# NTT123/vietTTS

Hardware: AMD Instinct MI355X
Metric: audio samples/sec whole-node, HiFi-GAN V1 mel2wave (higher is better)
Workload: dtype bf16; 1 GPU; HiFi-GAN V1 generator, 64 utterances x 1024 mel frames per GPU per step (BASELINE configs[2] shape), bf16; batch_per_gpu=64, frames=1024, parallelism=dp1 utterance-sharded, weights broadcast once, no data-path collective, microbatch=0, streams=0, schedule=engine default: micro-batches of <= 32768 frames on two HIP streams

## Files before the change

viettts_amd/csrc/engine.hip:

```cpp
#include "../../include/vtts_hifigan.h"

#include <hip/hip_runtime.h>

#include <cmath>
#include <cstdarg>
#include <cstdio>
#include <cstring>
#include <string>
#include <vector>

#include "vtts_internal.h"

using namespace vtts;

namespace {

thread_local std::string g_last_error;

}

int vtts::failf(int code, const char* fmt, ...) {
    char buf[512];
    va_list ap;
    va_start(ap, fmt);
    vsnprintf(buf, sizeof(buf), fmt, ap);
    va_end(ap);
    g_last_error = buf;
    return code;
}

namespace {

enum Kind { KIND_CONV = 0, KIND_CONVT = 1 };

struct Layer {
    std::string key;
    int kind = KIND_CONV;
    int cin = 0, cout = 0, k = 0, dil = 1, stride = 1;
    int pad = 0;
    int pad_a = 0;
    std::vector<float> w, b;
    bool have_w = false, have_b = false;
    size_t off_w = 0, off_b = 0, off_wp = 0;
    bool has_wp = false;
    size_t wp_floats = 0;
    int bcls = BCLS_NONE;
    size_t off_wb = 0, wb_bytes = 0;
    int coutp = 0;
    bool has_pair = false;
    size_t off_pw = 0, pw_bytes = 0, off_pb = 0;
    bool has_rb = false;
    size_t off_rw = 0, rw_bytes = 0, off_rb = 0;
    bool has_ug = false;
    size_t off_ug = 0, ug_bytes = 0;
    bool has_x3 = false;
    size_t off_x3 = 0;
};

}

struct vtts_hifigan {
    vtts_hifigan_cfg cfg;
    int device = 0;
    int dtype = VTTS_F32;
    bool x3 = false;
    int hop = 1;
    std::vector<Layer> layers;
    int idx_pre = -1, idx_post = -1;
    std::vector<int> idx_ups;
    std::vector<int> idx_res;
    size_t blob_bytes = 0;
    char* blob = nullptr;
    int64_t opt_kernels = 0;
    int64_t opt_microbatch = 0;
    int64_t opt_profile = 0;
    int cur_b0 = 0;
    const int* cur_lens = nullptr;
    int cur_T = 0;
    int64_t opt_tiles = 0;
    int64_t opt_fuse = 2;
    int64_t opt_streams = 0;
    int64_t opt_graph = 1;
    struct GraphEntry {
        const void* mel = nullptr;
        void* wav = nullptr;
        void* ws = nullptr;
        int B = 0, T = 0, seen = 0;
        uint64_t epoch = 0, last_use = 0;
        hipGraph_t graph = nullptr;
        hipGraphExec_t exec = nullptr;
    };
    std::vector<GraphEntry> graphs;
    hipStream_t cap_stream = nullptr;
    uint64_t epoch = 0, use_clock = 0;
    int64_t opt_zigzag = 1;
    unsigned zrev_count = 0;
    int64_t opt_tail = 1;
    int64_t opt_chains = 1;
    hipEvent_t ev_chain[3] = {nullptr, nullptr, nullptr};
    hipStream_t side_streams[3] = {nullptr, nullptr, nullptr};
    hipEvent_t ev_fork = nullptr, ev_join[3] = {nullptr, nullptr, nullptr};
    int prof_C = 0, prof_K = 0;
    std::vector<std::pair<hipEvent_t, hipEvent_t>> prof_events;
    size_t prof_used = 0;
    double prof_flops = 0.0;
    std::string prof_name, prof_name_pair;
};

namespace {

int conv_same_pad_a(int k, int s) {
    const int pad_len = k + s - 2;
    return (s > k - 1) ? (k - 1) : (pad_len + 1) / 2;
}

void pick_dominant_class(vtts_hifigan* h, bool mfma_only) {
    double best_flops = -1.0;
    for (const Layer& l : h->layers) {
        if (&l == &h->layers[h->idx_pre] || l.kind != KIND_CONV || l.cin != l.cout || (mfma_only && !l.has_wp)) continue;
        double fl = 0.0;
        long len2 = 1;
        for (auto& m : h->layers) {
            if (m.kind == KIND_CONVT) len2 *= m.stride;
            if (m.kind == KIND_CONV && m.cin == l.cin && m.k == l.k && m.cin == m.cout) fl += 2.0 * len2 * m.cin * m.cout * m.k;
        }
        if (fl > best_flops) {
            best_flops = fl;
            h->prof_C = l.cin;
            h->prof_K = l.k;
        }
    }
}

bool dominant(const vtts_hifigan* h, const Layer& l) {
    return l.kind == KIND_CONV && l.cin == h->prof_C && l.cout == h->prof_C && l.k == h->prof_K;
}

int classify_bf16(const vtts_hifigan* h, const Layer& l, bool is_pre, bool is_post) {
    if (is_post) return (l.cin == 32 && l.cout == 1 && l.k == 7) ? BCLS_NONE - 1 : BCLS_NONE;
    if (is_pre) return (l.cin <= 128 && l.cin % 8 == 0 && l.cout == 512 && l.k == 7) ? BCLS_PRE : BCLS_NONE;
    if (l.kind == KIND_CONVT) {
        if (!convT1d_f32_mfma_supported(l.cin, l.cout, l.k, l.stride, l.pad_a, 4)) return BCLS_NONE;
        if (l.cin == 512) return BCLS_UP0;
        if (l.cin == 256) return BCLS_UP1;
        if (l.cin == 128) return BCLS_UP2;
        return BCLS_UP3;
    }
    if (l.cin != l.cout || !(l.k == 3 || l.k == 7 || l.k == 11) || l.dil > 5) return BCLS_NONE;
    switch (l.cin) {
        case 256: return BCLS_RES256;
        case 128: return BCLS_RES128;
        case 64: return BCLS_RES64;
        case 32: return BCLS_RES32;
    }
    return BCLS_NONE;
}

int build_layers_bf16(vtts_hifigan* h) {
    size_t off = 0;
    for (auto& l : h->layers) {
        const bool is_pre = (&l == &h->layers[h->idx_pre]), is_post = (&l == &h->layers[h->idx_post]);
        l.bcls = classify_bf16(h, l, is_pre, is_post);
        if (l.bcls == BCLS_NONE)
            return failf(VTTS_ERR_INVALID, "dtype bf16: no kernel for module %s (%d->%d, k=%d): the bf16 path covers the HiFi-GAN V1 shapes",
                         l.key.c_str(), l.cin, l.cout, l.k);
        l.coutp = (l.kind == KIND_CONVT) ? l.cout * l.stride : l.cout;
        l.off_b = off;
        off = align_up(off + (size_t)l.coutp * sizeof(float), 256);
        if (is_post) {
            l.off_w = off;
            off = align_up(off + (size_t)l.k * l.cin * l.cout * sizeof(float), 256);
        } else {
            const BPackGeom g = bf16_pack_geom(l.bcls, l.kind == KIND_CONVT ? 3 : l.k);
            l.wb_bytes = bf16_packed_bytes(g);
            l.off_wb = off;
            off = align_up(off + l.wb_bytes, 256);
            if (l.kind == KIND_CONVT || (is_pre && l.bcls == BCLS_PRE && l.cin == 80)) {
                l.has_ug = true;
                l.ug_bytes = bf16_packed_bytes(convt_g_pack_geom(l.bcls));
                l.off_ug = off;
// ... 323 lines not shown
    const ConvArgs a = resblock_args(h, rb[0], x, B, L, y, acc_mode, div);
    const int dils[3] = {rb[0].dil, rb[2].dil, rb[4].dil};
    const void* w[6];
    const float* bias[6];
    for (int q = 0; q < 6; ++q) {
        w[q] = h->blob + rb[q].off_x3;
        bias[q] = reinterpret_cast<const float*>(h->blob + rb[q].off_b);
    }
    return launch_timed(h, rb[0], 6, B, L, s, "split-operand ResBlock launch", [&] { return launch_resblock_x3(a, dils, w, bias, s); });
}

int run_layer_bf16(vtts_hifigan* h, const Layer& l, const void* x, int x_pitch, int cin_real, int B, int L, float slope_in,
                   float slope_out, const void* res, void* y, int acc_add, float div, hipStream_t s) {
    BConvArgs a;
    memset(&a, 0, sizeof(a));
    a.x = x;
    a.wp = h->blob + l.off_wb;
    a.bias = reinterpret_cast<const float*>(h->blob + l.off_b);
    a.res = res;
    a.y = y;
    a.B = B;
    a.L = L;
    set_ragged(h, a, L);
    a.x_pitch = x_pitch;
    a.cin_real = cin_real;
    a.dil = (l.kind == KIND_CONVT) ? 1 : l.dil;
    a.pad = (l.kind == KIND_CONVT) ? 1 : l.pad;
    a.convt_halves = (l.kind == KIND_CONVT) ? 1 : 0;
    a.slope_in = slope_in;
    a.slope_out = slope_out;
    a.acc_add = acc_add;
    a.div = div;
    const int K = (l.kind == KIND_CONVT) ? 3 : l.k;
    const bool ug = (l.kind == KIND_CONVT || l.bcls == BCLS_PRE) && l.has_ug && h->opt_fuse >= 1 && res == nullptr && acc_add == 0 && div == 1.0f;
    if (ug) a.wp = h->blob + l.off_ug;
    if (ug) a.zrev = next_zrev(h);
    return launch_timed(h, l, 1, B, L, s, "bf16 kernel launch",
                        [&] { return ug ? launch_convt_g_bf16(l.bcls, a, s) : launch_conv_bf16(l.bcls, K, a, s); });
}

BConvArgs resblock_args_bf16(vtts_hifigan* h, const Layer& c1, const void* x, int B, int L, float slope_out, void* y, int acc_add, float div) {
    BConvArgs a;
    memset(&a, 0, sizeof(a));
    a.x = x;
    a.y = y;
    a.B = B;
    a.L = L;
    set_ragged(h, a, L);
    a.x_pitch = c1.cin;
    a.cin_real = c1.cin;
    a.slope_in = 0.1f;
    a.slope_out = slope_out;
    a.acc_add = acc_add;
    a.div = div;
    a.zrev = next_zrev(h);
    return a;
}

int run_pair_bf16(vtts_hifigan* h, const Layer& c1, const void* x, int B, int L, float slope_out, void* y, int acc_add, float div,
                  hipStream_t s, float* tail_wav = nullptr) {
    BConvArgs a = resblock_args_bf16(h, c1, x, B, L, slope_out, y, acc_add, div);
    a.wp = h->blob + c1.off_pw;
    a.bias = reinterpret_cast<const float*>(h->blob + c1.off_pb);
    a.dil = c1.dil;
    a.pad = c1.pad;
    a.tile_pref = (int)h->opt_tiles;
    if (tail_wav) {
        const Layer& post = h->layers[h->idx_post];
        a.tail_wav = tail_wav;
        a.tail_wf = reinterpret_cast<const float*>(h->blob + post.off_w);
        a.tail_bias = reinterpret_cast<const float*>(h->blob + post.off_b);
    }
    return launch_timed(h, c1, 2, B, L, s, "fused pair launch", [&] { return launch_pair_g_bf16(c1.cin, c1.k, a, s); });
}

int run_resblock_bf16(vtts_hifigan* h, const Layer* rb, const void* x, int B, int L, float slope_out, void* y, int acc_add, float div,
                      hipStream_t s) {
    BConvArgs a = resblock_args_bf16(h, rb[0], x, B, L, slope_out, y, acc_add, div);
    a.wp = h->blob + rb[0].off_rw;
    a.bias = reinterpret_cast<const float*>(h->blob + rb[0].off_rb);
    a.dils[0] = rb[0].dil;
    a.dils[1] = rb[2].dil;
    a.dils[2] = rb[4].dil;
    return launch_timed(h, rb[0], 0, B, L, s, "fused ResBlock launch", [&] { return launch_resblock_bf16(rb[0].cin, rb[0].k, a, s); });
}

Route route_bf16(const vtts_hifigan* h, const Layer* rb) {
    if (h->opt_fuse >= 2 && rb[0].has_rb && (h->opt_fuse >= 3 || resblock_bf16_preferred(rb[0].cin, rb[0].k))) return ROUTE_RESBLOCK;
    if (h->opt_fuse >= 1 && rb[0].has_pair && rb[2].has_pair && rb[4].has_pair) return ROUTE_PAIRS;
    return ROUTE_CONVS;
}

bool tail_fused_bf16(const vtts_hifigan* h) {
    if (!h->opt_tail || h->cfg.resblock == 2) return false;
    const Layer* rb = &h->layers[h->idx_res.back()];
    const Layer& post = h->layers[h->idx_post];
    return route_bf16(h, rb) == ROUTE_PAIRS && pair_tail_bf16_supported(rb[0].cin, rb[0].k, post.cin, post.cout, post.k);
}

size_t elem_bytes(const vtts_hifigan* h) { return h->dtype == VTTS_BF16 ? 2 : sizeof(float); }

size_t max_act_elems(const vtts_hifigan* h, int T) {
    size_t best = (size_t)h->cfg.upsample_initial_channel * T;
    long L = T;
    for (int i = 0; i < h->cfg.num_upsamples; ++i) {
        L *= h->cfg.upsample_rates[i];
        size_t e = (size_t)(h->cfg.upsample_initial_channel >> (i + 1)) * L;
        if (e > best) best = e;
    }
    return best;
}

int auto_streams(const vtts_hifigan* h) { return h->opt_streams > 0 ? (int)h->opt_streams : 2; }

int pass_frames(const vtts_hifigan* h) { return (h->dtype == VTTS_F32 && auto_streams(h) >= 2) ? 32768 : 65536; }

int microbatch_frames(const vtts_hifigan* h) { return auto_streams(h) >= 2 ? 32768 : 65536; }

int pick_microbatch(const vtts_hifigan* h, int B, int T) {
    if (h->opt_microbatch > 0) return (int)std::min<int64_t>(h->opt_microbatch, B);
    const int frames = microbatch_frames(h);
    int mb = (frames + T - 1) / T;
    if (mb < 1) mb = 1;
    if (mb > B) mb = B;
    int nmb = (B + mb - 1) / mb;
    const int ns = auto_streams(h);
    if (nmb > 1 && ns > 1) nmb = (nmb + ns - 1) / ns * ns;
    if (nmb > B) nmb = B;
    mb = (B + nmb - 1) / nmb;
    return mb;
}

int check_pass_size(const vtts_hifigan* h, int B, int T) {
    const size_t bytes = max_act_elems(h, T) * elem_bytes(h);
    if (bytes >= ((size_t)1 << 31))
        return failf(VTTS_ERR_INVALID, "T=%d frames is too long for one pass (%zu activation bytes per utterance, limit 2^31): synthesize it in chunks",
                     T, bytes);
    if (pick_microbatch(h, B, T) > 65535) return failf(VTTS_ERR_INVALID, "at most 65535 utterances per pass (got %d)", B);
    return VTTS_OK;
}

constexpr int PAR_CHAIN_FRAMES = 2048;

struct PassBufs {
    char *X = nullptr, *S = nullptr;
    char *T[VTTS_MAX_KERNELS] = {}, *C[VTTS_MAX_KERNELS] = {}, *Y[VTTS_MAX_KERNELS] = {};
};

struct PassPlan {
    int mb = 1, nstr = 1, nbuf = 4;
    size_t es = 0, per = 0;
    bool par = false;
    int chain_bufs = 0;

    size_t bytes() const { return (size_t)nstr * nbuf * per; }
    PassBufs buffers(void* ws, int si, int nk) const {
        char* slot = static_cast<char*>(ws) + (size_t)si * nbuf * per;
        auto at = [&](int q) { return slot + (size_t)q * per; };
        PassBufs b;
        b.X = at(0);
        b.S = at(par ? 1 : 3);
        for (int j = 0; j < nk; ++j) {
            b.T[j] = par ? at(2 + chain_bufs * j) : at(1);
            b.C[j] = par ? at(3 + chain_bufs * j) : at(2);
            if (par && chain_bufs == 3) b.Y[j] = at(4 + 3 * j);
        }
        return b;
// ... 649 lines not shown
    }
};

VTTS_API int vtts_hifigan_run_module(vtts_hifigan* h, const char* key, const float* x_dev, int B, int L, float slope_in,
                                     const float* res_dev, float* y_dev, vtts_stream stream) {
    if (!h || !key || !x_dev || !y_dev) return failf(VTTS_ERR_INVALID, "null argument");
    if (!h->blob) return failf(VTTS_ERR_STATE, "run_module() before pack()/bind_packed()");
    if (B <= 0 || L <= 0) return failf(VTTS_ERR_INVALID, "B and L must be positive");
    Layer* l = find_layer(h, key);
    if (!l) return failf(VTTS_ERR_INVALID, "unknown module '%s'", key);
    const bool is_pre = (l == &h->layers[h->idx_pre]);
    const bool is_post = (l == &h->layers[h->idx_post]);
    if (h->dtype == VTTS_BF16) {
        if (!(slope_in > 0.0f && slope_in <= 1.0f)) return failf(VTTS_ERR_INVALID, "run_module(): slope_in must lie in (0, 1] on a bf16 handle (got %g)", slope_in);
        hipStream_t st = static_cast<hipStream_t>(stream);
        const size_t nx = (size_t)B * L * l->cin, ny = (size_t)B * L * (l->kind == KIND_CONVT ? l->stride : 1) * l->cout;
        DevBuf xbuf, rbuf, ybuf;
        void *&xb = xbuf.p, *&rb = rbuf.p, *&yb = ybuf.p;
        int rc = VTTS_OK;
        if (is_post) {
            HIP_TRY(hipMalloc(&xb, nx * 2));
            if (launch_f32_to_bf16(x_dev, xb, nx, st) != hipSuccess) rc = failf(VTTS_ERR_HIP, "conversion launch failed");
            BConvArgs a;
            memset(&a, 0, sizeof(a));
            a.x = xb;
            a.wf = reinterpret_cast<const float*>(h->blob + l->off_w);
            a.bias = reinterpret_cast<const float*>(h->blob + l->off_b);
            a.B = B;
            a.L = L;
            if (!rc && launch_conv_post_bf16(a, y_dev, nullptr, st) != hipSuccess) rc = failf(VTTS_ERR_HIP, "conv_post launch failed");
        } else {
            HIP_TRY(hipMalloc(&yb, ny * 2));
            if (!is_pre) {
                HIP_TRY(hipMalloc(&xb, nx * 2));
                if (launch_f32_to_bf16(x_dev, xb, nx, st) != hipSuccess) rc = failf(VTTS_ERR_HIP, "conversion launch failed");
            }
            if (res_dev) {
                HIP_TRY(hipMalloc(&rb, ny * 2));
                if (launch_f32_to_bf16(res_dev, rb, ny, st) != hipSuccess) rc = failf(VTTS_ERR_HIP, "conversion launch failed");
            }
            if (!rc) rc = run_layer_bf16(h, *l, is_pre ? static_cast<const void*>(x_dev) : xb, l->cin, l->cin, B, L, slope_in, 1.0f, rb, yb, 0, 1.f, st);
            if (!rc && launch_bf16_to_f32(yb, y_dev, ny, st) != hipSuccess) rc = failf(VTTS_ERR_HIP, "conversion launch failed");
        }
        hipError_t e = hipStreamSynchronize(st);
        if (!rc && e != hipSuccess) rc = failf(VTTS_ERR_HIP, "run_module failed: %s", hipGetErrorString(e));
        return rc;
    }
    Act x = is_pre ? Act{x_dev, (long)L * l->cin, 1, l->cin} : Act{x_dev, (long)l->cin * L, L, 1};
    return run_layer(h, *l, x, B, L, slope_in, res_dev, y_dev, ACC_STORE, 1.f, is_post ? 1 : 0, nullptr,
                     static_cast<hipStream_t>(stream));
}

VTTS_API int vtts_hifigan_run_pair(vtts_hifigan* h, const char* key_c1, const float* x_dev, int B, int L, float* y_dev, vtts_stream stream) {
    if (!h || !key_c1 || !x_dev || !y_dev) return failf(VTTS_ERR_INVALID, "null argument");
    if (!h->blob) return failf(VTTS_ERR_STATE, "run_pair() before pack()/bind_packed()");
    if (B <= 0 || L <= 0) return failf(VTTS_ERR_INVALID, "B and L must be positive");
    Layer* l = find_layer(h, key_c1);
    const Layer* c2 = l && l + 1 < h->layers.data() + h->layers.size() ? l + 1 : nullptr;
    if (h->dtype == VTTS_F32) {
        const bool x3 = c2 && pair_x3_wanted(h, *l, *c2, L);
        if (!x3 && (!c2 || !pair_f32_fusable(*l, *c2, L)))
            return failf(VTTS_ERR_INVALID, "'%s' is not the first convolution of a ResBlock pair the fused fp32 kernel covers (C in {32, 64, 128}, L a multiple of 4)", key_c1);
        return run_pair_f32(h, *l, *c2, x3, x_dev, B, L, y_dev, ACC_STORE, 1.f, static_cast<hipStream_t>(stream));
    }
    if (!l || !l->has_pair) return failf(VTTS_ERR_INVALID, "'%s' is not the first convolution of a fused ResBlock pair", key_c1);
    hipStream_t st = static_cast<hipStream_t>(stream);
    const size_t n = (size_t)B * L * l->cin;
    DevBuf xbuf, ybuf;
    void *&xb = xbuf.p, *&yb = ybuf.p;
    HIP_TRY(hipMalloc(&xb, n * 2));
    HIP_TRY(hipMalloc(&yb, n * 2));
    int rc = VTTS_OK;
    if (launch_f32_to_bf16(x_dev, xb, n, st) != hipSuccess) rc = failf(VTTS_ERR_HIP, "conversion launch failed");
    if (!rc) rc = run_pair_bf16(h, *l, xb, B, L, 1.0f, yb, 0, 1.f, st);
    if (!rc && launch_bf16_to_f32(yb, y_dev, n, st) != hipSuccess) rc = failf(VTTS_ERR_HIP, "conversion launch failed");
    hipError_t e = hipStreamSynchronize(st);
    if (!rc && e != hipSuccess) rc = failf(VTTS_ERR_HIP, "run_pair failed: %s", hipGetErrorString(e));
    return rc;
}

VTTS_API int vtts_hifigan_set_option(vtts_hifigan* h, const char* name, int64_t value) {
    if (!h || !name) return failf(VTTS_ERR_INVALID, "null argument");
    {
        static const char* const writable[] = {"kernels", "microbatch", "fuse", "streams", "graph", "zigzag", "chains", "tiles", "tail", "stage"};
        for (const char* w : writable) {
            int64_t cur = 0;
            if (!strcmp(name, w) && vtts_hifigan_get_option(h, name, &cur) == VTTS_OK && cur == value) return VTTS_OK;
        }
    }
    ++h->epoch;
    if (!strcmp(name, "kernels")) {
        if (value != 0 && value != 1) return failf(VTTS_ERR_INVALID, "kernels must be 0 (auto) or 1 (generic)");
        h->opt_kernels = value;
    } else if (!strcmp(name, "microbatch")) {
        if (value < 0) return failf(VTTS_ERR_INVALID, "microbatch must be >= 0");
        h->opt_microbatch = value;
    } else if (!strcmp(name, "fuse")) {
        if (value < 0 || value > 3) return failf(VTTS_ERR_INVALID, "fuse must be 0 (per convolution), 1 (pairs), 2 (bf16: pairs + whole ResBlocks where faster; fp32: pairs at C <= 64) or 3 (... wherever supported)");
        h->opt_fuse = value;
    } else if (!strcmp(name, "streams")) {
        if (value < 0 || value > 4) return failf(VTTS_ERR_INVALID, "streams must be 1..4 (0 = the engine's default)");
        h->opt_streams = value;
    } else if (!strcmp(name, "graph")) {
        if (value != 0 && value != 1) return failf(VTTS_ERR_INVALID, "graph must be 0 (always eager) or 1 (small launches replay a captured hipGraph)");
        h->opt_graph = value;
    } else if (!strcmp(name, "zigzag")) {
        if (value != 0 && value != 1) return failf(VTTS_ERR_INVALID, "zigzag must be 0 or 1");
        h->opt_zigzag = value;
    } else if (!strcmp(name, "chains")) {
        if (value < 0 || value > 2) return failf(VTTS_ERR_INVALID, "chains must be 0 (ResBlocks of a stage one after the other), 1 (side by side on small fp32 launches) or 2 (... on every single-micro-batch launch)");
        h->opt_chains = value;
    } else if (!strcmp(name, "tiles")) {
        if (value < 0 || value > 2) return failf(VTTS_ERR_INVALID, "tiles must be 0 (auto), 1 (wide) or 2 (narrow)");
        h->opt_tiles = value;
    } else if (!strcmp(name, "tail")) {
        if (value != 0 && value != 1) return failf(VTTS_ERR_INVALID, "tail must be 0 or 1");
        h->opt_tail = value;
    } else if (!strcmp(name, "stage")) {
        if (value != 0) return failf(VTTS_ERR_INVALID, "stage must be 0: the whole-stage kernel was removed (it measured slower, profiles/r06_a_stage_kernel_findings.md)");
    } else if (!strcmp(name, "profile")) {
        h->opt_profile = value ? 1 : 0;
    } else if (!strcmp(name, "hop") || !strcmp(name, "pass_frames") || !strcmp(name, "max_frames_per_pass") || !strcmp(name, "graphs_cached") ||
               !strcmp(name, "profile_C") || !strcmp(name, "profile_K")) {
        return failf(VTTS_ERR_INVALID, "option '%s' is read-only", name);
    } else {
        return failf(VTTS_ERR_INVALID, "unknown option '%s'", name);
    }
    return VTTS_OK;
}

VTTS_API int vtts_hifigan_get_option(const vtts_hifigan* h, const char* name, int64_t* value) {
    if (!h || !name || !value) return failf(VTTS_ERR_INVALID, "null argument");
    if (!strcmp(name, "kernels")) *value = h->opt_kernels;
    else if (!strcmp(name, "microbatch")) *value = h->opt_microbatch;
    else if (!strcmp(name, "profile")) *value = h->opt_profile;
    else if (!strcmp(name, "tiles")) *value = h->opt_tiles;
    else if (!strcmp(name, "streams")) *value = h->opt_streams;
    else if (!strcmp(name, "zigzag")) *value = h->opt_zigzag;
    else if (!strcmp(name, "chains")) *value = h->opt_chains;
    else if (!strcmp(name, "graph")) *value = h->opt_graph;
    else if (!strcmp(name, "tail")) *value = h->opt_tail;
    else if (!strcmp(name, "stage")) *value = 0;
    else if (!strcmp(name, "graphs_cached")) {
        *value = 0;
        for (auto& g : h->graphs) *value += g.exec ? 1 : 0;
    }
    else if (!strcmp(name, "fuse")) *value = h->opt_fuse;
    else if (!strcmp(name, "hop")) *value = h->hop;
    else if (!strcmp(name, "max_frames_per_pass")) {
        const size_t per = max_act_elems(h, 1) * elem_bytes(h);
        *value = (int64_t)((((size_t)1 << 31) + per - 1) / per);
    }
    else if (!strcmp(name, "pass_frames")) *value = pass_frames(h);
    else if (!strcmp(name, "profile_C")) *value = h->prof_C;
    else if (!strcmp(name, "profile_K")) *value = h->prof_K;
    else return failf(VTTS_ERR_INVALID, "unknown option '%s'", name);
    return VTTS_OK;
}

VTTS_API int vtts_hifigan_profile_read(vtts_hifigan* h, double* resblock_ms, int64_t* launches, double* resblock_flops,
                                       int reset) {
    if (!h) return failf(VTTS_ERR_INVALID, "null argument");
    double ms = 0.0;
    for (size_t i = 0; i < h->prof_used; ++i) {
        float t = 0.f;
        HIP_TRY(hipEventSynchronize(h->prof_events[i].second));
        HIP_TRY(hipEventElapsedTime(&t, h->prof_events[i].first, h->prof_events[i].second));
        ms += t;
    }
    if (resblock_ms) *resblock_ms = ms;
    if (launches) *launches = (int64_t)h->prof_used;
    if (resblock_flops) *resblock_flops = h->prof_flops;
    if (reset) {
        h->prof_used = 0;
        h->prof_flops = 0.0;
    }
    return VTTS_OK;
}

VTTS_API const char* vtts_hifigan_profile_kernel(const vtts_hifigan* h) {
    if (!h) return "";
    return (h->dtype == VTTS_BF16 && h->opt_fuse) ? h->prof_name_pair.c_str() : h->prof_name.c_str();
}
```

viettts_amd/csrc/kernels_bf16_rbk.hip:

```cpp
#include <string.h>

#include <type_traits>

#include "bf16_common.h"

#ifndef VTTS_WREG_RB_MAX
#define VTTS_WREG_RB_MAX 64
#endif

namespace vtts {

template <int C_, int KS_, int W_, int WM_, int WN_, int PA_, int MINWG_>
struct RBTile {
    static constexpr int C = C_, KS = KS_, W = W_, WM = WM_, WN = WN_, PA = PA_, MINWG = MINWG_;
    static constexpr int THREADS = 64 * WM * WN, MR = C / WM / 32, NR = W / WN / 32;
    static constexpr int H = (KS - 1) / 2;
    static constexpr int MAXDIL = 5;
    static constexpr int GUARD = H * MAXDIL;
    static constexpr int ROWS = W + 2 * GUARD;
    static constexpr int SPR = C / 8, P = C * 2;
    static constexpr int KSTEPS = C / 16;
    static constexpr int NQT = KS * KSTEPS;
    static constexpr int MB = C / 32;
    static constexpr int RA = PA + 1;
    static constexpr int TILE_BYTES = tile_rows16(ROWS) * P;
    static constexpr int BIAS_BYTES = 6 * C * 4;
    static constexpr int LDS_BYTES = 2 * TILE_BYTES + BIAS_BYTES;
    static constexpr size_t CONV_BYTES = (size_t)KS * C * C * 2;
    static constexpr int XPT = (W * SPR + THREADS - 1) / THREADS;
    static_assert(C % (WM * 32) == 0 && W % (WN * 32) == 0 && LDS_BYTES <= 160 * 1024, "window / LDS");
    static_assert(RA == 4 && (NQT % 4 == 0 || NQT % 4 == 2), "ring of 4; a phase starts at slot 0 or 2");
    static constexpr bool WREG = NQT * MR * 4 <= VTTS_WREG_RB_MAX;
};

template <class T>
__global__ __launch_bounds__(T::THREADS, (T::MINWG * T::THREADS + 255) / 256) void resblock_bf16_k(BConvArgs a) {
    constexpr int C = T::C, KS = T::KS, W = T::W, PA = T::PA, RA = T::RA, MR = T::MR, NR = T::NR, H = T::H, GUARD = T::GUARD;
    constexpr int THREADS = T::THREADS, SPR = T::SPR, P = T::P, KSTEPS = T::KSTEPS, NQT = T::NQT, XPT = T::XPT, MB = T::MB;

    extern __shared__ __attribute__((aligned(16))) unsigned char lds[];
    unsigned char* tA = lds;
    unsigned char* tT = lds + T::TILE_BYTES;
    const float* sbias = reinterpret_cast<const float*>(lds + 2 * T::TILE_BYTES);

    const int tid = threadIdx.x;
    const int lane = tid & 63;
    const int wave = tid >> 6;
    const int wm = wave / T::WN, wn = wave % T::WN;
    const int cb0 = wm * (C / T::WM);
    const int l31 = lane & 31;
    const int lh = lane >> 5;
    const int b = a.zrev ? (int)(gridDim.z - 1 - blockIdx.z) : (int)blockIdx.z;
    const int Lp = a.L;
    const int L = a.lens ? min(max(a.lens[b], 0) * a.len_mul, a.L) : a.L;
    const int d0 = a.dils[0], d1 = a.dils[1], d2 = a.dils[2];
    const int M = H * (d0 + d1 + d2) + 3 * H;
    const int NT = W - 2 * M;
    const int ntv = (L + NT - 1) / NT, rx = (int)((blockIdx.x + b) & 7), lox = (rx * ntv) >> 3, hix = ((rx + 1) * ntv) >> 3;
    const bool xmap = (a.L + NT - 1) / NT >= 192;
    const int tile = xmap ? lox + (int)(blockIdx.x >> 3) : (int)blockIdx.x;
    if (xmap && tile >= hix) return;
    const int t0 = tile * NT;
    if (t0 >= L) return;
    const int tw = t0 - M;
    const unsigned short* __restrict__ xg = static_cast<const unsigned short*>(a.x) + (size_t)b * Lp * C;
    unsigned short* __restrict__ yg = static_cast<unsigned short*>(a.y) + (size_t)b * Lp * C;

    auto act2 = [](unsigned u) { return lrelu01_pack(bf16_lo(u), bf16_hi(u)); };

    for (int u = tid; u < 6 * C; u += THREADS) reinterpret_cast<float*>(lds + 2 * T::TILE_BYTES)[u] = a.bias[u];
    for (int u = tid; u < 2 * 2 * GUARD * SPR; u += THREADS) {
        const int tile = u / (2 * GUARD * SPR), v = u % (2 * GUARD * SPR);
        const int gr = v % (2 * GUARD), c = v / (2 * GUARD);
        const int row = gr < GUARD ? gr : W + gr;
        *reinterpret_cast<uint4*>((tile ? tT : tA) + tile_off<SPR>(row, c)) = make_uint4(0u, 0u, 0u, 0u);
    }
    {
        constexpr int RPI = THREADS / SPR;
        static_assert(THREADS % SPR == 0 && RPI % 16 == 0 && (W * SPR) % THREADS == 0, "a thread's units share their column and their swizzle");
        constexpr int RW = 64 / SPR;
        const int r0 = SPR >= 16 ? tid / SPR : wave * RW + lane % RW, c = SPR >= 16 ? tid % SPR : lane / RW;
        unsigned char* const lds0 = tA + tile_off<SPR>(GUARD + r0, c);
        uint4 v[XPT];
        if (tw >= 0 && tw + W <= L) {
            const unsigned short* __restrict__ g0 = xg + (size_t)(tw + r0) * C + c * 8;
#pragma unroll
            for (int i = 0; i < XPT; ++i) v[i] = *reinterpret_cast<const uint4*>(g0 + (size_t)i * RPI * C);
        } else {
#pragma unroll
            for (int i = 0; i < XPT; ++i) {
                const int t = tw + r0 + i * RPI;
                const int tc = t < 0 ? 0 : (t >= L ? L - 1 : t);
                v[i] = *reinterpret_cast<const uint4*>(xg + (size_t)tc * C + c * 8);
                if (t < 0 || t >= L) v[i] = make_uint4(0u, 0u, 0u, 0u);
            }
        }
#pragma unroll
        for (int i = 0; i < XPT; ++i) {
            v[i].x = act2(v[i].x);
            v[i].y = act2(v[i].y);
            v[i].z = act2(v[i].z);
            v[i].w = act2(v[i].w);
        }
#pragma unroll
        for (int i = 0; i < XPT; ++i) *reinterpret_cast<uint4*>(lds0 + i * RPI * P) = v[i];
    }
    const int col0 = wn * (W / T::WN) + l31;
    uint4 xr[MR][NR][2];
#pragma unroll
    for (int mr = 0; mr < MR; ++mr)
#pragma unroll
        for (int nr = 0; nr < NR; ++nr)
#pragma unroll
            for (int p = 0; p < 2; ++p) {
                const int t = tw + col0 + nr * 32;
// ... 61 lines not shown
            }
        };
        constexpr int TAILQ = NQT % 4;
        load_b(0, 0);
        __builtin_amdgcn_sched_group_barrier(0x100, NR, 0);
#pragma nounroll
        for (int q0 = 0; q0 < NQT - 4 - TAILQ; q0 += 4) {
#pragma unroll
            for (int i = 0; i < 4; ++i) step(q0 + i, i, true);
        }
        if constexpr (TAILQ == 0) {
#pragma unroll
            for (int i = 0; i < 4; ++i) step(NQT - 4 + i, i, i < 3);
        } else {
#pragma unroll
            for (int i = 0; i < 4; ++i) step(NQT - 6 + i, i, true);
            step(NQT - 2, 0, true);
            step(NQT - 1, 1, false);
        }
    };
    constexpr int NQW = T::WREG ? NQT : 1;
    bf16x8 aw[NQW][MR];
    auto load_w_all = [&](int conv) {
        if constexpr (T::WREG) {
            if (conv < 6) {
#pragma unroll
                for (int q = 0; q < NQT; ++q)
#pragma unroll
                    for (int mr = 0; mr < MR; ++mr) aw[q][mr] = __builtin_bit_cast(bf16x8, aptr[(size_t)((conv * NQT + q) * MB + mr) * 64]);
            }
        }
    };
    auto conv_phase_wreg = [&](const unsigned char* __restrict__ tile, int dl, int conv) {
        f32x16 bblk[MR];
#pragma unroll
        for (int mr = 0; mr < MR; ++mr)
#pragma unroll
            for (int rq = 0; rq < 4; ++rq) {
                const float4 bv = *reinterpret_cast<const float4*>(sbias + conv * C + cb0 + 32 * mr + 8 * rq + 4 * lh);
                bblk[mr][4 * rq + 0] = bv.x;
                bblk[mr][4 * rq + 1] = bv.y;
                bblk[mr][4 * rq + 2] = bv.z;
                bblk[mr][4 * rq + 3] = bv.w;
            }
        bf16x8 bf[2][NR];
        auto load_b = [&](int q, int par) {
            const int tap = q / KSTEPS, ks = q % KSTEPS;
#pragma unroll
            for (int nr = 0; nr < NR; ++nr) bf[par][nr] = *reinterpret_cast<const bf16x8*>(tile + tile_off<SPR>(GUARD + col0 + nr * 32 + (tap - H) * dl, ks * 2 + lh));
        };
        load_b(0, 0);
        __builtin_amdgcn_sched_group_barrier(0x100, NR, 0);
#pragma unroll
        for (int q = 0; q < NQT; ++q) {
            if (q + 1 < NQT) load_b(q + 1, (q + 1) & 1);
#pragma unroll
            for (int mr = 0; mr < MR; ++mr)
#pragma unroll
                for (int nr = 0; nr < NR; ++nr)
                    acc[mr][nr] = __builtin_amdgcn_mfma_f32_32x32x16_bf16(aw[q < NQW ? q : 0][mr], bf[q & 1][nr], q == 0 ? bblk[mr] : acc[mr][nr], 0, 0, 0);
            for (int i = 0; i < MR * NR; ++i) {
                __builtin_amdgcn_sched_group_barrier(0x008, 1, 0);
                if (q + 1 < NQT && i < NR) __builtin_amdgcn_sched_group_barrier(0x100, 1, 0);
            }
        }
    };
    if constexpr (T::WREG) {
        load_w_all(0);
    } else {
#pragma unroll
        for (int q = 0; q < PA; ++q) load_a(q, q % RA);
    }
    const bool interior = tw >= 0 && tw + W <= L;
    auto write_tile = [&](unsigned char* tile, int mr, int nr, unsigned p0, unsigned p1, unsigned q0, unsigned q1, int p) {
        const int row = GUARD + col0 + nr * 32;
        const int t = tw + col0 + nr * 32;
        if (!interior && (t < 0 || t >= L)) p0 = p1 = q0 = q1 = 0u;
        swap_pair(p0, q0);
        swap_pair(p1, q1);
        const int slot = ((cb0 + 32 * mr) >> 3) + 2 * p + lh;
        *reinterpret_cast<uint4*>(tile + tile_off<SPR>(row, slot)) = make_uint4(p0, p1, q0, q1);
    };

    __syncthreads();
    if constexpr (!T::WREG) init_acc(0);

    constexpr int S2 = NQT % 4;
#pragma nounroll
    for (int pr = 0; pr < 3; ++pr) {
        const int dl = pr == 0 ? d0 : (pr == 1 ? d1 : d2);
        if constexpr (T::WREG) {
            conv_phase_wreg(tA, dl, 2 * pr);
            load_w_all(2 * pr + 1);
        } else {
            conv_phase(2 * pr, std::integral_constant<int, 0>{}, tA, dl);
        }
#pragma unroll
        for (int mr = 0; mr < MR; ++mr)
#pragma unroll
            for (int nr = 0; nr < NR; ++nr)
#pragma unroll
                for (int p = 0; p < 2; ++p) {
                    const int r0 = 8 * p;
                    const f32x16& c = acc[mr][nr];
                    write_tile(tT, mr, nr, lrelu01_pack(c[r0 + 0], c[r0 + 1]), lrelu01_pack(c[r0 + 2], c[r0 + 3]),
                               lrelu01_pack(c[r0 + 4], c[r0 + 5]), lrelu01_pack(c[r0 + 6], c[r0 + 7]), p);
                }
        if constexpr (!T::WREG) init_acc(2 * pr + 1);
        __syncthreads();
        if constexpr (T::WREG) {
            conv_phase_wreg(tT, 1, 2 * pr + 1);
            load_w_all(2 * pr + 2);
        } else {
            conv_phase(2 * pr + 1, std::integral_constant<int, S2>{}, tT, 1);
        }
#pragma unroll
        for (int mr = 0; mr < MR; ++mr)
#pragma unroll
            for (int nr = 0; nr < NR; ++nr)
#pragma unroll
                for (int p = 0; p < 2; ++p) {
                    const int r0 = 8 * p;
                    const uint4 r = xr[mr][nr][p];
                    f32x16& c = acc[mr][nr];
                    c[r0 + 0] = vadd_raw(bf16_lo(r.x), c[r0 + 0]); c[r0 + 1] = vadd_raw(bf16_hi(r.x), c[r0 + 1]);
                    c[r0 + 2] = vadd_raw(bf16_lo(r.y), c[r0 + 2]); c[r0 + 3] = vadd_raw(bf16_hi(r.y), c[r0 + 3]);
                    c[r0 + 4] = vadd_raw(bf16_lo(r.z), c[r0 + 4]); c[r0 + 5] = vadd_raw(bf16_hi(r.z), c[r0 + 5]);
                    c[r0 + 6] = vadd_raw(bf16_lo(r.w), c[r0 + 6]); c[r0 + 7] = vadd_raw(bf16_hi(r.w), c[r0 + 7]);
                }
        if (pr < 2) {
#pragma unroll
            for (int mr = 0; mr < MR; ++mr)
#pragma unroll
                for (int nr = 0; nr < NR; ++nr)
#pragma unroll
                    for (int p = 0; p < 2; ++p) {
                        const int r0 = 8 * p;
                        const f32x16& c = acc[mr][nr];
                        uint4 r;
                        r.x = pack_bf16x2(c[r0 + 0], c[r0 + 1]);
                        r.y = pack_bf16x2(c[r0 + 2], c[r0 + 3]);
                        r.z = pack_bf16x2(c[r0 + 4], c[r0 + 5]);
                        r.w = pack_bf16x2(c[r0 + 6], c[r0 + 7]);
                        xr[mr][nr][p] = r;
                        write_tile(tA, mr, nr, act2(r.x), act2(r.y), act2(r.z), act2(r.w), p);
                    }
            if constexpr (!T::WREG) init_acc(2 * pr + 2);
            __syncthreads();
        }
    }

    {
        const float s_out = a.slope_out;
        const float dv = a.div;
        const float rdv = mrf_recip(dv);
        const bool acc_add = a.acc_add != 0;
        if (acc_add) {
#pragma unroll
            for (int mr = 0; mr < MR; ++mr)
#pragma unroll
                for (int nr = 0; nr < NR; ++nr)
#pragma unroll
                    for (int p = 0; p < 2; ++p) {
                        const int t = tw + col0 + nr * 32;
                        const int tc = t < 0 ? 0 : (t >= L ? L - 1 : t);
                        xr[mr][nr][p] = *reinterpret_cast<const uint4*>(yg + (size_t)tc * C + cb0 + 32 * mr + 16 * p + 8 * lh);
                    }
        }
#pragma unroll
        for (int mr = 0; mr < MR; ++mr)
#pragma unroll
            for (int nr = 0; nr < NR; ++nr)
#pragma unroll
                for (int p = 0; p < 2; ++p) {
                    const int n = col0 + nr * 32;
                    const int t = tw + n;
                    const bool ok = n >= M && n < W - M && t >= 0 && t < L;
                    const int r0 = 8 * p;
                    float v[8];
#pragma unroll
                    for (int e = 0; e < 8; ++e) v[e] = acc[mr][nr][r0 + e];
                    if (acc_add) {
                        uint4 o = xr[mr][nr][p];
                        swap_pair(o.x, o.z);
                        swap_pair(o.y, o.w);
                        v[0] = vadd_raw(bf16_lo(o.x), v[0]); v[1] = vadd_raw(bf16_hi(o.x), v[1]); v[2] = vadd_raw(bf16_lo(o.y), v[2]); v[3] = vadd_raw(bf16_hi(o.y), v[3]);
                        v[4] = vadd_raw(bf16_lo(o.z), v[4]); v[5] = vadd_raw(bf16_hi(o.z), v[5]); v[6] = vadd_raw(bf16_lo(o.w), v[6]); v[7] = vadd_raw(bf16_hi(o.w), v[7]);
                    }
                    if (dv != 1.0f) {
#pragma unroll
                        for (int e = 0; e < 8; ++e) v[e] = v[e] * rdv;
                    }
                    if (s_out != 1.0f) {
#pragma unroll
                        for (int e = 0; e < 8; ++e) v[e] = lrelu_f(v[e], s_out);
                    }
                    unsigned p0 = pack_bf16x2(v[0], v[1]), p1 = pack_bf16x2(v[2], v[3]);
                    unsigned q0 = pack_bf16x2(v[4], v[5]), q1 = pack_bf16x2(v[6], v[7]);
                    swap_pair(p0, q0);
                    swap_pair(p1, q1);
                    if (ok) *reinterpret_cast<uint4*>(yg + (size_t)t * C + cb0 + 32 * mr + 16 * p + 8 * lh) = make_uint4(p0, p1, q0, q1);
                }
    }
}

#ifndef VTTS_RB32_W
#define VTTS_RB32_W 512
#define VTTS_RB32_WN 4
#define VTTS_RB32_WG 2
#endif
#ifndef VTTS_RB64_W
#define VTTS_RB64_W 256
#define VTTS_RB64_WN 4
#define VTTS_RB64_WG 2
#endif
#ifndef VTTS_RB32K3_W
#define VTTS_RB32K3_W 256
#define VTTS_RB32K3_WG 3
#endif
template <int KS> using RB32 = RBTile<32, KS, KS == 3 ? VTTS_RB32K3_W : VTTS_RB32_W, 1, VTTS_RB32_WN, 3, KS == 3 ? VTTS_RB32K3_WG : VTTS_RB32_WG>;
template <int KS> using RB64 = RBTile<64, KS, VTTS_RB64_W, 1, VTTS_RB64_WN, 3, VTTS_RB64_WG>;
#ifndef VTTS_RB128_W
#define VTTS_RB128_W 128
#define VTTS_RB128_WN 2
#define VTTS_RB128_WG 2
#endif
template <int KS> using RB128 = RBTile<128, KS, VTTS_RB128_W, 2, VTTS_RB128_WN, 3, VTTS_RB128_WG>;
constexpr bool RB64_ALL_K = RB64<11>::LDS_BYTES * VTTS_RB64_WG <= 160 * 1024 && VTTS_RB64_W - 2 * 60 >= 128;

template <class T>
static hipError_t launch_rb(const BConvArgs& a, hipStream_t s) {
    static DynLdsOnce once;
    if (hipError_t e = set_max_dynamic_lds(reinterpret_cast<const void*>(&resblock_bf16_k<T>), T::LDS_BYTES, once); e != hipSuccess) return e;
    int dsum = 0;
    for (int i = 0; i < 3; ++i) {
        if (a.dils[i] < 1 || a.dils[i] > T::MAXDIL) return hipErrorInvalidValue;
        dsum += a.dils[i];
    }
    const int NT = T::W - 2 * (T::H * dsum + 3 * T::H);
    if (NT < 32) return hipErrorInvalidValue;
    dim3 grid((a.L + NT - 1) / NT, 1, a.B);
    if ((int)grid.x >= 192) grid.x = (grid.x + 7) / 8 * 8;
    hipLaunchKernelGGL(resblock_bf16_k<T>, grid, dim3(T::THREADS), T::LDS_BYTES, s, a);
    return hipGetLastError();
}

bool resblock_bf16_supported(int C, int K, const int* dils) {
    for (int i = 0; i < 3; ++i)
        if (dils[i] < 1 || dils[i] > 5) return false;
    if (C == 32) return K == 3 || K == 7 || K == 11;
    if (C == 64 && RB64_ALL_K) return K == 3 || K == 7 || K == 11;
    return (C == 64 || C == 128) && K == 3;
}
bool resblock_bf16_preferred(int C, int K) { return (C == 32 && (K == 3 || K == 7)) || (C == 64 && K == 3); }

hipError_t launch_resblock_bf16(int C, int K, const BConvArgs& a, hipStream_t s) {
    if (C == 32) switch (K) {
            case 3: return launch_rb<RB32<3>>(a, s);
            case 7: return launch_rb<RB32<7>>(a, s);
            case 11: return launch_rb<RB32<11>>(a, s);
        }
    if (C == 64 && K == 3) return launch_rb<RB64<3>>(a, s);
    if constexpr (RB64_ALL_K) {
        if (C == 64 && K == 7) return launch_rb<RB64<7>>(a, s);
        if (C == 64 && K == 11) return launch_rb<RB64<11>>(a, s);
    }
    if (C == 128 && K == 3) return launch_rb<RB128<3>>(a, s);
    return hipErrorInvalidValue;
}

}
```

viettts_amd/csrc/vtts_internal.h:

```cpp
#pragma once

#include <hip/hip_runtime.h>
#include <stddef.h>
#include <stdint.h>
#include <string.h>

#include "../../include/vtts_hifigan.h"

#define VTTS_API extern "C" __attribute__((visibility("default")))

namespace vtts {

int failf(int code, const char* fmt, ...);

#define HIP_TRY(expr)                                                                                          \
    do {                                                                                                       \
        hipError_t _e = (expr);                                                                                \
        if (_e != hipSuccess)                                                                                  \
            return vtts::failf(VTTS_ERR_HIP, "%s failed: %s (%s:%d)", #expr, hipGetErrorString(_e), __FILE__, __LINE__); \
    } while (0)

inline size_t align_up(size_t v, size_t a) { return (v + a - 1) / a * a; }

inline int check_blob(const void* dev_blob, size_t bytes, size_t need) {
// ... 84 lines not shown
void pair_x3_pack(const float* w_hk, int C, int K, unsigned short* out);
hipError_t launch_pair_x3(const ConvArgs& a, const void* w1, const void* w2, const float* bias2, hipStream_t s);
bool convt_x3_supported(int Cin, int Cout, int K, int stride, int pad_a, int L);
size_t convt_x3_bytes(int Cin, int Cout, int stride);
void convt_x3_pack(const float* w_hk, int Cin, int Cout, int K, int stride, int pad_a, unsigned short* out);
hipError_t launch_convt_x3(const ConvArgs& a, hipStream_t s);
bool conv_pre_x3_supported(int Cin, int Cout, int K, int dil);
size_t conv_pre_x3_bytes();
void conv_pre_x3_pack(const float* w_hk, unsigned short* out);
hipError_t launch_conv_pre_x3(const ConvArgs& a, hipStream_t s);

bool resblock_x3_supported(int C, int K, const int* dils, int L);
bool resblock_x3_preferred(int C, int K);
hipError_t launch_resblock_x3(const ConvArgs& a, const int* dils, const void* const* w, const float* const* bias, hipStream_t s);

bool convT1d_f32_mfma_supported(int Cin, int Cout, int K, int stride, int pad_a, int L);
size_t convT1d_f32_mfma_packed_floats(int Cin, int Cout, int K);
void convT1d_f32_mfma_pack(const float* w_hk, int Cin, int Cout, int K, int stride, int pad_a, float* out);
hipError_t launch_convT1d_f32_mfma(const ConvArgs& a, hipStream_t s);

bool conv_post_fast_supported(int Cin, int Cout, int K, int L);
hipError_t launch_conv_post_fast(const ConvArgs& a, hipStream_t s);

enum BClass : int { BCLS_NONE = -1, BCLS_RES256 = 0, BCLS_RES128, BCLS_RES64, BCLS_RES32, BCLS_PRE, BCLS_UP0, BCLS_UP1, BCLS_UP2, BCLS_UP3 };

struct BConvArgs {
    const void* x;
    const void* wp;
    const float* wf;
    const float* bias;
    const void* res;
    void* y;
    int B, L;
    const int* lens;
    int len_mul;
    int x_pitch;
    int cin_real;
    int dil, pad;
    int convt_halves;
    int dils[3];
    float slope_in;
    float slope_out;
    int acc_add;
    int tile_pref;
    float div;
    int zrev;
    unsigned long long* dbg;
    float* tail_wav;
    const float* tail_wf;
    const float* tail_bias;
};

struct BPackGeom { int cinp, ckc, coutp, ks, mt, tg; };

hipError_t launch_conv_bf16(int cls, int K, const BConvArgs& a, hipStream_t s);
BPackGeom bf16_pack_geom(int cls, int K);
const char* bf16_kernel_name(int cls, int K);
inline size_t bf16_packed_bytes(const BPackGeom& g) {
    const int ncc = g.cinp / g.ckc, nsl = (g.ks + g.tg - 1) / g.tg;
    return (size_t)(g.coutp / g.mt) * ncc * nsl * ((size_t)g.mt * g.tg * g.ckc * 2);
}
void bf16_pack(const float* Wc, int cin_real, const BPackGeom& g, unsigned short* out);
bool pair_bf16_supported(int C, int K, int dil);
bool pair_tail_bf16_supported(int C, int K, int post_cin, int post_cout, int post_k);
hipError_t launch_pair_g_bf16(int C, int K, const BConvArgs& a, hipStream_t s);
BPackGeom pair_g_pack_geom(int C, int K);
int pair_g_mfma_blk(int C, int K);
inline size_t pair_g_pack16_bytes(int C, int K) { return (size_t)K * (C / 32) * (C / 16) * 64 * 8 * sizeof(unsigned short); }
inline void pair_g_pack16(const float* Wc, int C, int K, unsigned short* out) {
    size_t o = 0;
    for (int tap = 0; tap < K; ++tap)
        for (int ks = 0; ks < C / 32; ++ks)
            for (int mblk = 0; mblk < C / 16; ++mblk)
                for (int lane = 0; lane < 64; ++lane)
                    for (int e = 0; e < 8; ++e) {
                        const int ci = 32 * ks + 8 * (lane >> 4) + e, co = 16 * mblk + (lane & 15);
                        out[o++] = f32_to_bf16_rne(Wc[((size_t)tap * C + ci) * C + co]);
                    }
}
void pair_g_pack(const float* Wc, int C, int K, unsigned short* out);
const char* pair_g_kernel_name(int C, int K);
bool resblock_bf16_supported(int C, int K, const int* dils);
bool resblock_bf16_preferred(int C, int K);
hipError_t launch_resblock_bf16(int C, int K, const BConvArgs& a, hipStream_t s);
hipError_t launch_convt_g_bf16(int cls, const BConvArgs& a, hipStream_t s);
BPackGeom convt_g_pack_geom(int cls);
hipError_t launch_conv_post_bf16(const BConvArgs& a, float* wav, float* pre_act, hipStream_t s);
hipError_t launch_bf16_to_f32(const void* in, float* out, size_t n, hipStream_t s);
hipError_t launch_f32_to_bf16(const float* in, void* out, size_t n, hipStream_t s);


constexpr int NAT_RES_H = 512, NAT_RES_PN = 256, NAT_RES_MELMAX = 128;
constexpr int NAT_RES_XCH_ELEMS = NAT_RES_MELMAX + 2 * NAT_RES_PN + 2 * NAT_RES_H;
struct NatResidentArgs {
    const float* w1;
    const float* w2;
    const float* wp;
    const float* bp;
    const float* f1;
    const float* f2;
    const float* G1;
    const float* G2;
    const int* nframes;
    const unsigned char* keep;
    float* mel0;
    float* xch;
    unsigned* sync;
    unsigned long long* timeline;
    int Fmax, MEL;
};
hipError_t launch_nat_dec_resident(const NatResidentArgs& a, int B, int grid, hipStream_t s);

}
```

Before: 437.5 million samples/s.

## Split fused C=32 K=7 ResBlock conv phases into column-block halves to overlap epilogues

Adds a split variant of the fused bf16 ResBlock kernel for C=32, K=7. Each convolution phase is computed in two halves: first the inner column blocks (1,2), whose epilogue is written to LDS, then the edge blocks (0,3) while the next conv's weights are loaded into registers. The aim is to shorten barrier stalls and overlap epilogue and weight-load work with MFMA work. A new 'split' option, on by default, selects it. The cost is more code, higher register pressure and an extra __syncthreads per half-phase.

```diff
diff --git a/viettts_amd/csrc/engine.hip b/viettts_amd/csrc/engine.hip
--- a/viettts_amd/csrc/engine.hip
+++ b/viettts_amd/csrc/engine.hip
@@ -96,6 +96,7 @@
     int64_t opt_zigzag = 1;
     unsigned zrev_count = 0;
     int64_t opt_tail = 1;
+    int64_t opt_split = 1;
     int64_t opt_chains = 1;
     hipEvent_t ev_chain[3] = {nullptr, nullptr, nullptr};
     hipStream_t side_streams[3] = {nullptr, nullptr, nullptr};
@@ -585,7 +586,7 @@
     a.dils[0] = rb[0].dil;
     a.dils[1] = rb[2].dil;
     a.dils[2] = rb[4].dil;
-    return launch_timed(h, rb[0], 0, B, L, s, "fused ResBlock launch", [&] { return launch_resblock_bf16(rb[0].cin, rb[0].k, a, s); });
+    return launch_timed(h, rb[0], 0, B, L, s, "fused ResBlock launch", [&] { return launch_resblock_bf16(rb[0].cin, rb[0].k, a, s, (int)h->opt_split); });
 }
 
 Route route_bf16(const vtts_hifigan* h, const Layer* rb) {
@@ -1401,7 +1402,7 @@
 VTTS_API int vtts_hifigan_set_option(vtts_hifigan* h, const char* name, int64_t value) {
     if (!h || !name) return failf(VTTS_ERR_INVALID, "null argument");
     {
-        static const char* const writable[] = {"kernels", "microbatch", "fuse", "streams", "graph", "zigzag", "chains", "tiles", "tail", "stage"};
+        static const char* const writable[] = {"kernels", "microbatch", "fuse", "streams", "graph", "zigzag", "chains", "tiles", "tail", "split", "stage"};
         for (const char* w : writable) {
             int64_t cur = 0;
             if (!strcmp(name, w) && vtts_hifigan_get_option(h, name, &cur) == VTTS_OK && cur == value) return VTTS_OK;
@@ -1435,6 +1436,9 @@
     } else if (!strcmp(name, "tail")) {
         if (value != 0 && value != 1) return failf(VTTS_ERR_INVALID, "tail must be 0 or 1");
         h->opt_tail = value;
+    } else if (!strcmp(name, "split")) {
+        if (value != 0 && value != 1) return failf(VTTS_ERR_INVALID, "split must be 0 or 1");
+        h->opt_split = value;
     } else if (!strcmp(name, "stage")) {
         if (value != 0) return failf(VTTS_ERR_INVALID, "stage must be 0: the whole-stage kernel was removed (it measured slower, profiles/r06_a_stage_kernel_findings.md)");
     } else if (!strcmp(name, "profile")) {
@@ -1459,6 +1463,7 @@
     else if (!strcmp(name, "chains")) *value = h->opt_chains;
     else if (!strcmp(name, "graph")) *value = h->opt_graph;
     else if (!strcmp(name, "tail")) *value = h->opt_tail;
+    else if (!strcmp(name, "split")) *value = h->opt_split;
     else if (!strcmp(name, "stage")) *value = 0;
     else if (!strcmp(name, "graphs_cached")) {
         *value = 0;
diff --git a/viettts_amd/csrc/kernels_bf16_rbk.hip b/viettts_amd/csrc/kernels_bf16_rbk.hip
--- a/viettts_amd/csrc/kernels_bf16_rbk.hip
+++ b/viettts_amd/csrc/kernels_bf16_rbk.hip
@@ -31,6 +31,13 @@
     static_assert(C % (WM * 32) == 0 && W % (WN * 32) == 0 && LDS_BYTES <= 160 * 1024, "window / LDS");
     static_assert(RA == 4 && (NQT % 4 == 0 || NQT % 4 == 2), "ring of 4; a phase starts at slot 0 or 2");
     static constexpr bool WREG = NQT * MR * 4 <= VTTS_WREG_RB_MAX;
+    static constexpr bool SPLIT = false;
+};
+
+template <class B>
+struct RBSplit : B {
+    static constexpr bool SPLIT = true;
+    static_assert(B::WREG && B::NR == 4 && B::GUARD < 32, "four column blocks per wave, taps within one block, weights in registers");
 };
 
 template <class T>
@@ -258,6 +265,84 @@
         *reinterpret_cast<uint4*>(tile + tile_off<SPR>(row, slot)) = make_uint4(p0, p1, q0, q1);
     };
 
+    [[maybe_unused]] auto conv_part_wreg = [&](auto b0_tag, auto b1_tag, auto next_tag, const unsigned char* __restrict__ tile, int dl, int conv) {
+        constexpr int BLKS[2] = {decltype(b0_tag)::value, decltype(b1_tag)::value};
+        constexpr bool NEXT = decltype(next_tag)::value;
+        const int cn = conv + 1 < 6 ? conv + 1 : 5;
+        f32x16 bblk[MR];
+#pragma unroll
+        for (int mr = 0; mr < MR; ++mr)
+#pragma unroll
+            for (int rq = 0; rq < 4; ++rq) {
+                const float4 bv = *reinterpret_cast<const float4*>(sbias + conv * C + cb0 + 32 * mr + 8 * rq + 4 * lh);
+                bblk[mr][4 * rq + 0] = bv.x;
+                bblk[mr][4 * rq + 1] = bv.y;
+                bblk[mr][4 * rq + 2] = bv.z;
+                bblk[mr][4 * rq + 3] = bv.w;
+            }
+        bf16x8 bf[2][2];
+        auto load_b = [&](int q, int par) {
+            const int tap = q / KSTEPS, ks = q % KSTEPS;
+#pragma unroll
+            for (int i = 0; i < 2; ++i) bf[par][i] = *reinterpret_cast<const bf16x8*>(tile + tile_off<SPR>(GUARD + col0 + BLKS[i] * 32 + (tap - H) * dl, ks * 2 + lh));
+        };
+        load_b(0, 0);
+        __builtin_amdgcn_sched_barrier(0);
+#pragma unroll
+        for (int q = 0; q < NQT; ++q) {
+            if (q + 1 < NQT) load_b(q + 1, (q + 1) & 1);
+#pragma unroll
+            for (int mr = 0; mr < MR; ++mr)
+#pragma unroll
+                for (int i = 0; i < 2; ++i)
+                    acc[mr][BLKS[i]] = __builtin_amdgcn_mfma_f32_32x32x16_bf16(aw[q < NQW ? q : 0][mr], bf[q & 1][i], q == 0 ? bblk[mr] : acc[mr][BLKS[i]], 0, 0, 0);
+            for (int i = 0; i < MR * 2; ++i) {
+                __builtin_amdgcn_sched_group_barrier(0x008, 1, 0);
+                if (q + 1 < NQT && i < 2) __builtin_amdgcn_sched_group_barrier(0x100, 1, 0);
+            }
+            if constexpr (NEXT) {
+                __builtin_amdgcn_sched_barrier(0);
+#pragma unroll
+                for (int mr = 0; mr < MR; ++mr) aw[q < NQW ? q : 0][mr] = __builtin_bit_cast(bf16x8, aptr[(size_t)((cn * NQT + q) * MB + mr) * 64]);
+            }
+            __builtin_amdgcn_sched_barrier(0);
+        }
+    };
+    [[maybe_unused]] auto ep1_block = [&](int nr) {
+#pragma unroll
+        for (int mr = 0; mr < MR; ++mr)
+#pragma unroll
+            for (int p = 0; p < 2; ++p) {
+                const int r0 = 8 * p;
+                const f32x16& c = acc[mr][nr];
+                write_tile(tT, mr, nr, lrelu01_pack(c[r0 + 0], c[r0 + 1]), lrelu01_pack(c[r0 + 2], c[r0 + 3]),
+                           lrelu01_pack(c[r0 + 4], c[r0 + 5]), lrelu01_pack(c[r0 + 6], c[r0 + 7]), p);
+            }
+    };
+    [[maybe_unused]] auto ep2_block = [&](int nr, bool more) {
+#pragma unroll
+        for (int mr = 0; mr < MR; ++mr)
+#pragma unroll
+            for (int p = 0; p < 2; ++p) {
+                const int r0 = 8 * p;
+                const uint4 o = xr[mr][nr][p];
+                f32x16& c = acc[mr][nr];
+                c[r0 + 0] = vadd_raw(bf16_lo(o.x), c[r0 + 0]); c[r0 + 1] = vadd_raw(bf16_hi(o.x), c[r0 + 1]);
+                c[r0 + 2] = vadd_raw(bf16_lo(o.y), c[r0 + 2]); c[r0 + 3] = vadd_raw(bf16_hi(o.y), c[r0 + 3]);
+                c[r0 + 4] = vadd_raw(bf16_lo(o.z), c[r0 + 4]); c[r0 + 5] = vadd_raw(bf16_hi(o.z), c[r0 + 5]);
+                c[r0 + 6] = vadd_raw(bf16_lo(o.w), c[r0 + 6]); c[r0 + 7] = vadd_raw(bf16_hi(o.w), c[r0 + 7]);
+                if (more) {
+                    uint4 r;
+                    r.x = pack_bf16x2(c[r0 + 0], c[r0 + 1]);
+                    r.y = pack_bf16x2(c[r0 + 2], c[r0 + 3]);
+                    r.z = pack_bf16x2(c[r0 + 4], c[r0 + 5]);
+                    r.w = pack_bf16x2(c[r0 + 6], c[r0 + 7]);
+                    xr[mr][nr][p] = r;
+                    write_tile(tA, mr, nr, act2(r.x), act2(r.y), act2(r.z), act2(r.w), p);
+                }
+            }
+    };
+
     __syncthreads();
     if constexpr (!T::WREG) init_acc(0);
 
@@ -265,6 +350,28 @@
 #pragma nounroll
     for (int pr = 0; pr < 3; ++pr) {
         const int dl = pr == 0 ? d0 : (pr == 1 ? d1 : d2);
+        if constexpr (T::SPLIT) {
+            using B0 = std::integral_constant<int, 0>;
+            using B1 = std::integral_constant<int, 1>;
+            using B2 = std::integral_constant<int, 2>;
+            using B3 = std::integral_constant<int, 3>;
+            const bool more = pr < 2;
+            conv_part_wreg(B1{}, B2{}, std::false_type{}, tA, dl, 2 * pr);
+            ep1_block(1);
+            ep1_block(2);
+            __syncthreads();
+            conv_part_wreg(B0{}, B3{}, std::true_type{}, tA, dl, 2 * pr);
+            ep1_block(0);
+            ep1_block(3);
+            conv_part_wreg(B1{}, B2{}, std::false_type{}, tT, 1, 2 * pr + 1);
+            ep2_block(1, more);
+            ep2_block(2, more);
+            __syncthreads();
+            conv_part_wreg(B0{}, B3{}, std::true_type{}, tT, 1, 2 * pr + 1);
+            ep2_block(0, more);
+            ep2_block(3, more);
+            continue;
+        }
         if constexpr (T::WREG) {
             conv_phase_wreg(tA, dl, 2 * pr);
             load_w_all(2 * pr + 1);
@@ -404,6 +511,8 @@
 template <int KS> using RB128 = RBTile<128, KS, VTTS_RB128_W, 2, VTTS_RB128_WN, 3, VTTS_RB128_WG>;
 constexpr bool RB64_ALL_K = RB64<11>::LDS_BYTES * VTTS_RB64_WG <= 160 * 1024 && VTTS_RB64_W - 2 * 60 >= 128;
 
+constexpr bool rb_split(int C, int KS) { return C == 32 && KS == 7; }
+
 template <class T>
 static hipError_t launch_rb(const BConvArgs& a, hipStream_t s) {
     static DynLdsOnce once;
@@ -430,10 +539,14 @@
 }
 bool resblock_bf16_preferred(int C, int K) { return (C == 32 && (K == 3 || K == 7)) || (C == 64 && K == 3); }
 
-hipError_t launch_resblock_bf16(int C, int K, const BConvArgs& a, hipStream_t s) {
+hipError_t launch_resblock_bf16(int C, int K, const BConvArgs& a, hipStream_t s, int split) {
     if (C == 32) switch (K) {
             case 3: return launch_rb<RB32<3>>(a, s);
-            case 7: return launch_rb<RB32<7>>(a, s);
+            case 7:
+                if constexpr (rb_split(32, 7)) {
+                    if (split) return launch_rb<RBSplit<RB32<7>>>(a, s);
+                }
+                return launch_rb<RB32<7>>(a, s);
             case 11: return launch_rb<RB32<11>>(a, s);
         }
     if (C == 64 && K == 3) return launch_rb<RB64<3>>(a, s);
diff --git a/viettts_amd/csrc/vtts_internal.h b/viettts_amd/csrc/vtts_internal.h
--- a/viettts_amd/csrc/vtts_internal.h
+++ b/viettts_amd/csrc/vtts_internal.h
@@ -190,7 +190,7 @@
 const char* pair_g_kernel_name(int C, int K);
 bool resblock_bf16_supported(int C, int K, const int* dils);
 bool resblock_bf16_preferred(int C, int K);
-hipError_t launch_resblock_bf16(int C, int K, const BConvArgs& a, hipStream_t s);
+hipError_t launch_resblock_bf16(int C, int K, const BConvArgs& a, hipStream_t s, int split = 1);
 hipError_t launch_convt_g_bf16(int cls, const BConvArgs& a, hipStream_t s);
 BPackGeom convt_g_pack_geom(int cls);
 hipError_t launch_conv_post_bf16(const BConvArgs& a, float* wav, float* pre_act, hipStream_t s);
```

Result: no change. 438.6 million samples/s, median of 6 (+0.3%).
